# QEDProtocol/plonky2.5

Hardware: AMD Instinct MI355X
Metric: recursive proofs/sec (fib-64 p3-in-p2 circuit) (higher is better)
Workload: dtype u64 (Goldilocks, p = 2^64 - 2^32 + 1); 1 GPU; batch of 256 independent fib-64 plonky3-verifier proofs per GPU (n = 2^16 rows x 135 wires, LDE 2^19), 1 GPU(s), replicas + RCCL gather; all_statuses_ok=True, gathered_complete_and_ok=True, head=

## Files before the change

### plonky2.5_amd/csrc/capi.hip

```cpp
#include <stdlib.h>
#include <dirent.h>
#include <unistd.h>
#include <cstring>
#include <memory>
#include <atomic>
#include <mutex>
#include "../../include/p25.h"
#include "kernels.h"
#include "circuit_io.h"
#include "circuit_bytes.h"
#include "json_io.h"
#include "p3_circuit.h"
#include "p3_prover.h"
#include "p3_kernels.h"
#include "prover.h"
#include "recursion.h"

namespace p25 {
thread_local std::string g_last_error;
static std::atomic<int> g_device{-1};
static std::once_flag g_tables_once;
static std::unique_ptr<NttTables> g_tables;
static std::mutex g_primitives_mutex;

// ... 343 lines not shown
    bits -= a;
    if (deg < 0 || bits < (int)cap_height) return false;
  }
  return true;
}
}
}

using namespace p25;

extern "C" {

const char* p25_last_error(void) { return g_last_error.c_str(); }
const char* p25_version(void) { return "libp25 0.1 (gfx950)"; }

p25_status p25_device_init(int device_index) {
  const p25_status s = p25_device_init_ex(device_index, P25_DEFAULT_HW_QUEUES);
  return s == P25_WARN_HW_QUEUES_LATE ? P25_OK : s;
}

p25_status p25_device_init_ex(int device_index, int hw_queues) {
  if (hw_queues < 0 || hw_queues > P25_DEFAULT_HW_QUEUES) {
    g_last_error = "hw_queues out of range (0..2; 0 = leave the runtime's setting alone)";
    return P25_ERR_INVALID_ARG;
  }
  const bool late = apply_hw_queues(hw_queues);
  int n = 0;
  if (hipGetDeviceCount(&n) != hipSuccess || n <= 0) {
    g_last_error = "no HIP device available (libp25 has no CPU fallback)";
    return P25_ERR_NO_DEVICE;
  }
  if (device_index < 0 || device_index >= n) {
    g_last_error = "device index out of range";
    return P25_ERR_INVALID_ARG;
  }
  if (hipSetDevice(device_index) != hipSuccess) {
    g_last_error = "hipSetDevice failed";
    return P25_ERR_HIP;
  }
  g_device.store(device_index, std::memory_order_release);
  if (late) {
    g_last_error = HWQ_LATE_MSG;
    return P25_WARN_HW_QUEUES_LATE;
  }
  return P25_OK;
}

p25_status p25_runtime_info(p25_runtime_info_t* out) {
  if (!out) {
    g_last_error = "out is null";
    return P25_ERR_INVALID_ARG;
  }
  memset(out, 0, sizeof *out);
  out->device_index = g_device.load(std::memory_order_acquire);
  {
    std::lock_guard<std::mutex> l(g_hwq.mu);
    out->hw_queues_requested = g_hwq.requested;
    out->hw_queues_host_exported = g_hwq.host_exported ? 1 : 0;
    out->runtime_open_before_init = g_hwq.runtime_was_up ? 1 : 0;
    out->hw_queues_setting_late = (g_hwq.decided && g_hwq.requested > 0 && !g_hwq.host_exported && g_hwq.runtime_was_up) ? 1 : 0;
  }
  const char* e = getenv("GPU_MAX_HW_QUEUES");
  out->hw_queues_env = e ? (int32_t)strtol(e, nullptr, 10) : 0;
  out->proving_streams = 16;
  out->main_streams = 2;
  return P25_OK;
}

p25_status p25_poseidon_permute(uint64_t* states, size_t n) { return permute_host(states, n, launch_poseidon_permute, true); }
p25_status p25_poseidon2_permute(uint64_t* states, size_t n) { return permute_host(states, n, launch_poseidon2_permute, false); }

p25_status p25_merkle_commit(const uint64_t* leaves_cm, size_t n_leaves, size_t width,
                             unsigned cap_height, uint64_t* cap_out, uint64_t* tree_out) {
  return guarded([&]() -> p25_status {
    if (!is_pow2(n_leaves) || cap_height > 40 || n_leaves < ((size_t)1 << cap_height) || !width ||
        width > (1u << 20) || !leaves_cm)
      throw std::invalid_argument("p25_merkle_commit: bad shape");
    for (size_t i = 0; i < n_leaves * width; i++)
      if (leaves_cm[i] >= gl::P) throw std::invalid_argument("p25_merkle_commit: non-canonical field element");
    DevBuf d(n_leaves * width);
    size_t tw = merkle_tree_words(n_leaves, cap_height);
    DevBuf t(tw);
    P25_HIP(hipMemcpy(d.p, leaves_cm, n_leaves * width * 8, hipMemcpyHostToDevice));
    u64* cap = launch_merkle_tree(d.p, n_leaves, (int)width, n_leaves, cap_height, t.p, 0);
    P25_HIP(hipGetLastError());
    if (cap_out) P25_HIP(hipMemcpy(cap_out, cap, ((size_t)32) << cap_height, hipMemcpyDeviceToHost));
    if (tree_out) P25_HIP(hipMemcpy(tree_out, t.p, tw * 8, hipMemcpyDeviceToHost));
    P25_HIP(hipDeviceSynchronize());
    return P25_OK;
  });
}
size_t p25_merkle_tree_words(size_t n_leaves, unsigned cap_height) {
  if (!is_pow2(n_leaves) || cap_height > 63 || n_leaves < ((size_t)1 << cap_height)) return 0;
  return merkle_tree_words(n_leaves, cap_height);
}
p25_status p25_lde_commit(const uint64_t* polys, unsigned log_n, size_t n_polys, int from_coeffs,
                          unsigned rate_bits, unsigned cap_height, uint64_t* coeffs_out,
                          uint64_t* lde_out, uint64_t* cap_out) {
  return guarded([&]() -> p25_status {
    if (!polys || !n_polys || log_n > 20 || rate_bits > 3 || log_n + rate_bits < cap_height)
      throw std::invalid_argument("p25_lde_commit: bad shape");
    const size_t n = (size_t)1 << log_n, big = n << rate_bits;
    for (size_t i = 0; i < n * n_polys; i++)
      if (polys[i] >= gl::P) throw std::invalid_argument("p25_lde_commit: non-canonical field element");
    std::lock_guard<std::mutex> lk(g_primitives_mutex);
    DevBuf in(n * n_polys), co(n * n_polys), tmp(n * n_polys), lde(big * n_polys);
    size_t tw = merkle_tree_words(big, cap_height);
    DevBuf tree(tw);
    P25_HIP(hipMemcpy(in.p, polys, n * n_polys * 8, hipMemcpyHostToDevice));
    lde_commit_dev(in.p, log_n, n_polys, from_coeffs != 0, rate_bits, cap_height, co.p, tmp.p, lde.p,
                   tree.p, 0);
    P25_HIP(hipGetLastError());
    P25_HIP(hipDeviceSynchronize());
    if (coeffs_out)
      P25_HIP(hipMemcpy(coeffs_out, from_coeffs ? in.p : co.p, n * n_polys * 8, hipMemcpyDeviceToHost));
    if (lde_out) P25_HIP(hipMemcpy(lde_out, lde.p, big * n_polys * 8, hipMemcpyDeviceToHost));
    if (cap_out)
      P25_HIP(hipMemcpy(cap_out, tree.p + tw - ((size_t)4 << cap_height), ((size_t)32) << cap_height,
                        hipMemcpyDeviceToHost));
    return P25_OK;
  });
}
p25_status p25_merkle_commit_dev(const uint64_t* d_leaves_cm, size_t col_stride, size_t n_leaves,
                                 size_t width, unsigned cap_height, uint64_t* d_tree, void* stream) {
  return guarded([&]() -> p25_status {
    if (width > (1u << 20)) throw std::invalid_argument("p25_merkle_commit_dev: width above 2^20");
    if (!is_pow2(n_leaves) || cap_height > 40 || n_leaves < ((size_t)1 << cap_height) || !width ||
        col_stride < n_leaves || !d_leaves_cm || !d_tree)
      throw std::invalid_argument("p25_merkle_commit_dev: bad shape");
    launch_merkle_tree(d_leaves_cm, col_stride, (int)width, n_leaves, cap_height, d_tree,
                       (hipStream_t)stream);
    P25_HIP(hipGetLastError());
    return P25_OK;
  });
}
p25_status p25_lde_commit_dev(const uint64_t* d_polys, unsigned log_n, size_t n_polys, int from_coeffs,
                              unsigned rate_bits, unsigned cap_height, uint64_t* d_coeffs,
                              uint64_t* d_tmp, uint64_t* d_lde, uint64_t* d_tree, void* stream) {
  return guarded([&]() -> p25_status {
    if (log_n <= 20 && rate_bits <= 3 && cap_height > log_n + rate_bits)
      throw std::invalid_argument("p25_lde_commit_dev: cap_height above log_n + rate_bits");
    if (!d_polys || !n_polys || log_n > 20 || rate_bits > 3 || !d_lde ||
        (!from_coeffs && (!d_coeffs || !d_tmp)))
      throw std::invalid_argument("p25_lde_commit_dev: bad shape");
    std::lock_guard<std::mutex> lk(g_primitives_mutex);
    lde_commit_dev(d_polys, log_n, n_polys, from_coeffs != 0, rate_bits, cap_height, d_coeffs, d_tmp,
                   d_lde, d_tree, (hipStream_t)stream);
    P25_HIP(hipGetLastError());
    return P25_OK;
  });
}
p25_status p25_poseidon_permute_dev(uint64_t* d_states, size_t n, void* stream) {
  return guarded([&]() -> p25_status {
    launch_poseidon_permute(d_states, n, (hipStream_t)stream);
    P25_HIP(hipGetLastError());
    return P25_OK;
  });
}

p25_status p25_circuit_build_p3_verifier(const p25_p3_config* cfg, int32_t air, p25_circuit** out) {
  return host_guarded([&]() -> p25_status {
    if (!cfg || !out) throw std::invalid_argument("null argument");
    if (air != P25_AIR_FIBONACCI) throw std::invalid_argument("unknown AIR");
    FibonacciAir fib;
    return build_verifier(cfg, fib, out);
  });
}
// ... 520 lines not shown
```

### plonky2.5_amd/csrc/kernels.h

```cpp
#pragma once
#include <hip/hip_runtime.h>
#include <stddef.h>
#include <stdint.h>
#include <stdexcept>
#include <string>
#include <vector>
#include <map>
#include <tuple>
#include "gl.h"

#if defined(__HIP_DEVICE_COMPILE__)
#define P25_WAVE_PRIO(n) __builtin_amdgcn_s_setprio(n)
#else
#define P25_WAVE_PRIO(n) ((void)0)
#endif
#define P25_PRIO_BULK 2
#define P25_PRIO_CHAIN 3
namespace p25 {

struct HipError : std::runtime_error {
  using std::runtime_error::runtime_error;
};
#define P25_HIP(expr)                                                                         \
  do {                                                                                        \
    hipError_t _e = (expr);                                                                   \
    if (_e != hipSuccess)                                                                     \
      throw p25::HipError(std::string(#expr) + ": " + hipGetErrorString(_e) + " at " +        \
                          __FILE__ + ":" + std::to_string(__LINE__));                         \
  } while (0)

void launch_poseidon_permute(u64* d_states, size_t n, hipStream_t st);
void launch_poseidon2_permute(u64* d_states, size_t n, hipStream_t st);
size_t merkle_tree_words(size_t n_leaves, unsigned cap_height);
size_t merkle_level_offset(size_t n_leaves, unsigned level);
u64* launch_merkle_tree(const u64* d_cols, size_t col_stride, int width, size_t n_leaves,
                        unsigned cap_height, u64* d_tree, hipStream_t st, hipEvent_t ev_begin = nullptr,
                        hipEvent_t ev_end = nullptr, bool single_proof = false);

struct NttPass {
  const u64* in;
  u64* out;
  size_t in_poly_stride, out_poly_stride;
  size_t coset_out_off[8];
  int log_r, log_nt, log_t;
  int in_kind, in_br_t, in_br_i;
  int out_kind, out_br_t, out_br_i;
  const u64* pow_table;
  int log_n_table;
  int use_twiddle;
  const u64* pre;
  const u64* pre_t;
  const u64* pre_i;
  const u64* post_t;
  const u64* post_i;
  int inverse;
  int lazy_out;
  uint32_t n_tiles, n_cosets, log_g, full_table;
};
void launch_ntt_pass(const NttPass& p, int n_polys, int n_cosets, hipStream_t st);
double measure_shader_clock_hz(hipStream_t st);

class NttTables {
 public:
  ~NttTables();
  const u64* pow_table(int log_n, bool inverse);
  const u64* geom_table(u64 first, u64 ratio, size_t len);
  const u64* upload(const std::vector<u64>& host);
  typedef std::map<std::tuple<int, int, u64>, const u64*> CosetCache;
  CosetCache& coset_cache() { return coset_; }

 private:
  CosetCache coset_;
  std::map<std::pair<int, bool>, u64*> pow_;
  std::map<std::tuple<u64, u64, size_t>, u64*> geom_;
  std::vector<u64*> owned_;
};

void ntt_inverse(NttTables& tb, const u64* d_in, size_t in_stride, bool in_bitrev, u64* d_tmp,
                 size_t tmp_stride, u64* d_out, size_t out_stride, int log_n, int n_polys,
                 u64 coset_shift, hipStream_t st);
void ntt_lde_bitrev(NttTables& tb, const u64* d_coeffs, size_t coeff_stride, u64* d_lde,
                    size_t lde_stride, int log_n, int rate_bits, int n_polys, u64 shift,
                    hipStream_t st);

void ntt_inverse_then_lde(NttTables& tb, const u64* d_vals, size_t val_stride, u64* d_tmp, size_t tmp_stride, u64* d_coeffs,
                          size_t coeff_stride, u64* d_lde, size_t lde_stride, int log_n, int rate_bits, int n_polys, u64 shift,
                          hipStream_t st);

}
```

### plonky2.5_amd/csrc/kernels_hash.hip

```cpp
#include "kernels.h"
#include "poseidon.h"
#include "poseidon2.h"
#include "coop.h"
#include "coop_lat.h"

namespace p25 {

__global__ __launch_bounds__(256) void k_poseidon_permute(u64* states, size_t n) {
  size_t i = (size_t)blockIdx.x * blockDim.x + threadIdx.x;
  if (i >= n) return;
  u64 s[12];
#pragma unroll
  for (int k = 0; k < 12; k++) s[k] = states[i * 12 + k];
  poseidon::permute(s);
#pragma unroll
  for (int k = 0; k < 12; k++) states[i * 12 + k] = s[k];
}

__global__ __launch_bounds__(256) void k_poseidon2_permute(u64* states, size_t n) {
  size_t i = (size_t)blockIdx.x * blockDim.x + threadIdx.x;
  if (i >= n) return;
  u64 s[12];
#pragma unroll
  for (int k = 0; k < 12; k++) s[k] = states[i * 12 + k];
  poseidon2::permute(s);
#pragma unroll
  for (int k = 0; k < 12; k++) states[i * 12 + k] = s[k];
}

__device__ __forceinline__ void hash_leaf(const u64* __restrict__ cols, size_t col_stride, int width,
                                          size_t n_leaves, u64* __restrict__ digests) {
  size_t l = (size_t)blockIdx.x * 64 + threadIdx.x;
  if (l >= n_leaves) return;
  u64 out[4];
  poseidon::hash_or_noop_strided(cols + l, col_stride, width, out);
  u64* d = digests + 4 * l;
#pragma unroll
  for (int i = 0; i < 4; i++) d[i] = out[i];
}
__global__ __launch_bounds__(64, 6) void k_hash_leaves(const u64* __restrict__ cols, size_t col_stride,
                                                       int width, size_t n_leaves, u64* __restrict__ digests) {
  hash_leaf(cols, col_stride, width, n_leaves, digests);
}
__global__ __launch_bounds__(64, 6) void k_hash_leaves_wide(const u64* __restrict__ cols, size_t col_stride,
                                                            int width, size_t n_leaves, u64* __restrict__ digests) {
  hash_leaf(cols, col_stride, width, n_leaves, digests);
}

template <int PRIO>
__global__ __launch_bounds__(64, 8) void k_tree_level(const u64* __restrict__ children,
                                                    u64* __restrict__ parents, size_t n_parents) {
  if constexpr (PRIO != 0) P25_WAVE_PRIO(PRIO);
  size_t m = (size_t)blockIdx.x * 64 + threadIdx.x;
  if (m >= n_parents) return;
  u64 l[4], r[4], o[4];
#pragma unroll
  for (int i = 0; i < 4; i++) {
    l[i] = children[8 * m + i];
    r[i] = children[8 * m + 4 + i];
  }
  poseidon::two_to_one(l, r, o);
#pragma unroll
  for (int i = 0; i < 4; i++) parents[4 * m + i] = o[i];
}

__global__ __launch_bounds__(256) void k_tree_level_coop(const u64* __restrict__ children,
                                                         u64* __restrict__ parents, size_t n_parents) {
  P25_WAVE_PRIO(P25_PRIO_CHAIN);
  __shared__ u64 rc_lds[360];
  coop::stage_poseidon_rc(rc_lds);
  size_t g = ((size_t)blockIdx.x * blockDim.x + threadIdx.x) / coop::GROUP;
  const int rr = threadIdx.x & (coop::GROUP - 1);
  const bool valid = g < n_parents;
  if (!valid) g = n_parents - 1;
  u64 s = rr < 8 ? children[8 * g + rr] : 0;
  s = coop::poseidon_permute_lat(s, threadIdx.x & 63, rc_lds);
  if (valid && rr < 4) parents[4 * g + rr] = s;
}
constexpr int TOP_GROUPS = 16;
constexpr size_t TOP_MAX_NODES = 2 * TOP_GROUPS;
__global__ __launch_bounds__(256) void k_tree_top_coop(u64* __restrict__ nodes, uint32_t per_block, uint32_t n_blocks) {
  P25_WAVE_PRIO(P25_PRIO_CHAIN);
  __shared__ u64 rc_lds[360];
  __shared__ u64 lvl[2][TOP_GROUPS * 4];
  coop::stage_poseidon_rc(rc_lds);
  const int g = threadIdx.x / coop::GROUP, rr = threadIdx.x & (coop::GROUP - 1), lane = threadIdx.x & 63;
  const uint32_t b = blockIdx.x;
  u64* cur = nodes;
  size_t level_nodes = (size_t)per_block * n_blocks;
  uint32_t np = per_block >> 1;
  int buf = 0;
  bool first = true;
  while (np >= 1) {
    u64* nxt = cur + 4 * level_nodes;
    const uint32_t j = (uint32_t)g < np ? (uint32_t)g : np - 1;
    if ((uint32_t)(g & ~3) < np) {
      u64 s = 0;
      if (rr < 8) s = first ? cur[4 * ((size_t)b * 2 * np) + 8 * j + rr] : lvl[buf ^ 1][8 * j + rr];
      s = coop::poseidon_permute_lat(s, lane, rc_lds);
      if ((uint32_t)g < np && rr < 4) {
        nxt[4 * ((size_t)b * np + j) + rr] = s;
        lvl[buf][4 * j + rr] = s;
      }
    }
    __syncthreads();
    cur = nxt;
    level_nodes >>= 1;
    np >>= 1;
    buf ^= 1;
    first = false;
  }
}

constexpr size_t COOP_PARENTS_BATCH = 2048, COOP_PARENTS_SINGLE = 32768;
constexpr int LEVEL_PRIO_BATCH = 1;

static void launch_level(const u64* cur, u64* nxt, size_t m, hipStream_t st, bool single_proof) {
  const dim3 grid((unsigned)((m + 63) / 64));
  if (m <= (single_proof ? COOP_PARENTS_SINGLE : COOP_PARENTS_BATCH)) {
    size_t th = m * coop::GROUP;
    hipLaunchKernelGGL(k_tree_level_coop, dim3((unsigned)((th + 255) / 256)), dim3(256), 0, st, cur, nxt, m);
  } else if (single_proof) {
    hipLaunchKernelGGL(k_tree_level<0>, grid, dim3(64), 0, st, cur, nxt, m);
  } else {
    hipLaunchKernelGGL(k_tree_level<LEVEL_PRIO_BATCH>, grid, dim3(64), 0, st, cur, nxt, m);
  }
}
static u64* launch_levels_to_cap(u64* cur, size_t m, unsigned cap_height, hipStream_t st, bool single_proof) {
  const size_t cap = (size_t)1 << cap_height;
  while (m > cap) {
    if (m / cap <= TOP_MAX_NODES && cap <= 65536) {
      hipLaunchKernelGGL(k_tree_top_coop, dim3((unsigned)cap), dim3(TOP_GROUPS * coop::GROUP), 0, st, cur,
                         (uint32_t)(m / cap), (uint32_t)cap);
      while (m > cap) {
        cur += 4 * m;
        m >>= 1;
      }
      return cur;
    }
    u64* nxt = cur + 4 * m;
    m >>= 1;
    launch_level(cur, nxt, m, st, single_proof);
    cur = nxt;
  }
  return cur;
}

__global__ __launch_bounds__(64) void k_clock_probe(u64* sink, int reps, unsigned long long* clk) {
  size_t l = (size_t)blockIdx.x * blockDim.x + threadIdx.x;
  u64 s[12];
#pragma unroll
  for (int i = 0; i < 12; i++) s[i] = l * 12 + i;
  unsigned long long c0 = __builtin_readcyclecounter(), w0 = wall_clock64();
  for (int r = 0; r < reps; r++) {
    s[0] ^= (u64)r;
    poseidon::permute(s);
  }
  unsigned long long c1 = __builtin_readcyclecounter(), w1 = wall_clock64();
  if (s[0] == 0x123456789ull) sink[l & 63] = s[1];
  if (threadIdx.x == 0 && (blockIdx.x & 1023) == 0) {
    clk[2 * (blockIdx.x >> 10)] = c1 - c0;
    clk[2 * (blockIdx.x >> 10) + 1] = w1 - w0;
  }
}
double measure_shader_clock_hz(hipStream_t st) {
  const unsigned blocks = 8192, probes = blocks / 1024;
  u64* d = nullptr;
  P25_HIP(hipMalloc(&d, (64 + 2 * probes) * 8));
  unsigned long long* clk = (unsigned long long*)(d + 64);
  int dev = 0, khz = 0;
  P25_HIP(hipGetDevice(&dev));
  P25_HIP(hipDeviceGetAttribute(&khz, hipDeviceAttributeWallClockRate, dev));
  unsigned long long h[2 * probes];
  for (int it = 0; it < 2; it++)
    hipLaunchKernelGGL(k_clock_probe, dim3(blocks), dim3(64), 0, st, d, 64, clk);
  hipError_t e = hipMemcpyAsync(h, clk, sizeof(h), hipMemcpyDeviceToHost, st);
  if (e == hipSuccess) e = hipStreamSynchronize(st);
  (void)hipFree(d);
  P25_HIP(e);
  double cyc = 0, ticks = 0;
  for (unsigned i = 0; i < probes; i++) {
    cyc += (double)h[2 * i];
    ticks += (double)h[2 * i + 1];
  }
  if (ticks <= 0 || khz <= 0) return 0.0;
  return cyc / (ticks / ((double)khz * 1e3));
}

void launch_poseidon_permute(u64* d_states, size_t n, hipStream_t st) {
  if (!n) return;
  hipLaunchKernelGGL(k_poseidon_permute, dim3((unsigned)((n + 255) / 256)), dim3(256), 0, st, d_states, n);
}
void launch_poseidon2_permute(u64* d_states, size_t n, hipStream_t st) {
  if (!n) return;
  hipLaunchKernelGGL(k_poseidon2_permute, dim3((unsigned)((n + 255) / 256)), dim3(256), 0, st, d_states, n);
}

size_t merkle_tree_words(size_t n_leaves, unsigned cap_height) {
  size_t total = 0;
  for (size_t m = n_leaves; m >= ((size_t)1 << cap_height); m >>= 1) {
    total += 4 * m;
    if (m == 1) break;
  }
  return total;
}
size_t merkle_level_offset(size_t n_leaves, unsigned level) {
  size_t off = 0;
  size_t m = n_leaves;
  for (unsigned k = 0; k < level; k++) {
    off += 4 * m;
    m >>= 1;
  }
  return off;
}

u64* launch_merkle_tree(const u64* d_cols, size_t col_stride, int width, size_t n_leaves,
                        unsigned cap_height, u64* d_tree, hipStream_t st, hipEvent_t ev_begin,
                        hipEvent_t ev_end, bool single_proof) {
  if (ev_begin) (void)hipEventRecord(ev_begin, st);
  if (width >= 128)
    hipLaunchKernelGGL(k_hash_leaves_wide, dim3((unsigned)((n_leaves + 63) / 64)), dim3(64), 0, st, d_cols,
                       col_stride, width, n_leaves, d_tree);
  else
    hipLaunchKernelGGL(k_hash_leaves, dim3((unsigned)((n_leaves + 63) / 64)), dim3(64), 0, st, d_cols,
                       col_stride, width, n_leaves, d_tree);
  if (ev_end) (void)hipEventRecord(ev_end, st);
  return launch_levels_to_cap(d_tree, n_leaves, cap_height, st, single_proof);
}

void launch_tree_from_digests(u64* d_tree, size_t n_leaves, unsigned cap_height, hipStream_t st, bool single_proof) {
  launch_levels_to_cap(d_tree, n_leaves, cap_height, st, single_proof);
}

}
```

### plonky2.5_amd/csrc/prover.hip

```cpp
#include "prover.h"
#include <algorithm>
#include <map>
#include <mutex>
#include <string.h>
#include "poseidon.h"

namespace p25 {

constexpr size_t STREAM_POOL = 16;
namespace {
struct StreamPool {
  std::mutex mu;
  std::map<int, std::vector<hipStream_t>> per_device;
  size_t cursor = 0;
  size_t width = STREAM_POOL;
  size_t reserve(size_t count, size_t want_width) {
    std::lock_guard<std::mutex> l(mu);
    if (want_width > width) width = want_width;
    size_t first = cursor % width;
    cursor += count;
    return first;
  }
  void widen(size_t want_width) {
    std::lock_guard<std::mutex> l(mu);
// ... 104 lines not shown
  size_t m = (size_t)1 << log_n;
  const size_t nl = arity_bits.size();
  if (nl > 8) throw std::invalid_argument("too many FRI layers");
  for (size_t l = 0; l <= nl; l++) {
    coeffs[l] = DevMem(2 * m);
    if (l < nl) {
      size_t nvals = m << rate_bits;
      vals[l] = DevMem(2 * nvals);
      tree[l] = DevMem(merkle_tree_words(nvals >> arity_bits[l], cap_height));
      m >>= arity_bits[l];
    }
  }
}

void fri_commit_pow_query(NttTables& tables, FriWork& w, const FriShape& sh, Transcript* tr, u64* chal, QueryArgs qy,
                          u64* d_proof, const FriOffsets& fo, uint32_t* d_status, hipStream_t st, bool single_proof) {
  const size_t capw = (size_t)4 << sh.cap_height;
  size_t m = (size_t)1 << sh.log_n;
  int log_m = sh.log_n;
  u64 shift = gl::GENERATOR;
  const size_t nl = sh.arity_bits.size();
  for (size_t l = 0; l < nl; l++) {
    const int ab = sh.arity_bits[l];
    const size_t nvals = m << sh.rate_bits;
    ntt_lde_bitrev(tables, w.coeffs[l].p, m, w.vals[l].p, nvals, log_m, sh.rate_bits, 2, shift, st);
    const size_t n_leaves = nvals >> ab;
    launch_fri_leaf_hash(w.vals[l].p, w.vals[l].p + nvals, (uint32_t)n_leaves, ab, w.tree[l].p, st, single_proof);
    launch_tree_from_digests(w.tree[l].p, n_leaves, sh.cap_height, st, single_proof);
    const size_t ltw = merkle_tree_words(n_leaves, sh.cap_height);
    const u64* cap = w.tree[l].p + ltw - capw;
    {
      TranscriptArgs ta{};
      ta.seg[0] = TrSegment{cap, nullptr, d_proof + fo.caps + l * capw, (uint32_t)capw};
      ta.n_seg = 1;
      ta.chal_out = chal + CH_FRI_BETAS + 2 * l;
      ta.n_chal = 2;
      launch_transcript(tr, ta, st);
    }
    launch_fri_fold(w.coeffs[l].p, w.coeffs[l].p + m, (uint32_t)(m >> ab), ab, chal + CH_FRI_BETAS + 2 * l,
                    w.coeffs[l + 1].p, w.coeffs[l + 1].p + (m >> ab), st);
    qy.arity_bits[l] = ab;
    qy.layer_va[l] = w.vals[l].p;
    qy.layer_vb[l] = w.vals[l].p + nvals;
    qy.layer_tree[l] = w.tree[l].p;
    shift = gl::pow(shift, (u64)1 << ab);
    m >>= ab;
    log_m -= ab;
  }
  {
    TranscriptArgs ta{};
    ta.seg[0] = TrSegment{w.coeffs[nl].p, w.coeffs[nl].p + m, d_proof + fo.final_poly, (uint32_t)(2 * m)};
    ta.n_seg = 1;
    ta.close = TR_CLOSE_POW_INIT;
    ta.close_out = chal + CH_POW_WITNESS;
    launch_transcript(tr, ta, st);
  }
  qy.n_layers = (uint32_t)nl;
  launch_pow_search(tr, sh.pow_bits, chal + CH_POW_WITNESS, st, single_proof);
  {
    TranscriptArgs ta{};
    ta.seg[0] = TrSegment{chal + CH_POW_WITNESS, nullptr, d_proof + fo.pow_witness, 1};
    ta.n_seg = 1;
    ta.chal_out = chal + CH_POW_RESPONSE;
    ta.n_chal = 1 + (uint32_t)sh.num_queries;
    ta.close = TR_CLOSE_FINISH;
    ta.close_arg = (uint32_t)sh.pow_bits;
    ta.status = d_status;
    launch_transcript(tr, ta, st);
  }
  qy.chal = chal;
  qy.num_queries = sh.num_queries;
  qy.lde_bits = sh.log_n + sh.rate_bits;
  qy.cap_height = sh.cap_height;
  qy.proof = d_proof;
  qy.query_offset = (uint32_t)fo.queries;
  qy.query_stride = (uint32_t)fo.query_stride;
  launch_queries(qy, st);
}

struct DeviceCircuit::Ctx {
  DevMem wires_vals, wires_coeffs, tmp, wires_lde, wires_tree;
  DevMem zs_vals, zs_coeffs, zs_lde, zs_tree, zpp_chunk, zpp_tot, zpp_btot;
  DevMem q_vals, q_tmp, q_coeffs, q_lde, q_tree;
  DevMem transcript, chal, alpha_pows, eval_pows;
  DevMem preamble;
  DevMem fri_comp, fri_scan;
  FriWork fri;
  DevMem proof, status;
  hipEvent_t ev[12];
  hipStream_t st = nullptr;
  hipEvent_t done[2] = {nullptr, nullptr};
  hipEvent_t join = nullptr;
  bool have_events = false;
  ~Ctx() {
    if (have_events)
      for (auto& e : ev) (void)hipEventDestroy(e);
    for (auto& e : done)
      if (e) (void)hipEventDestroy(e);
    if (join) (void)hipEventDestroy(join);
  }
};

DeviceCircuit::DeviceCircuit(Circuit c) : c_(std::move(c)) {
  if (c_.cfg.num_challenges != 2 || c_.cfg.rate_bits > 3 || c_.gates.size() > 16)
    throw std::invalid_argument("unsupported circuit configuration");
  if (c_.fri_reduction_arity_bits.size() > 8) throw std::invalid_argument("too many FRI layers");
  if (c_.num_partial_products + 1 > MAX_CHUNKS || c_.cfg.num_routed_wires > MAX_ROUTED ||
      c_.cfg.num_challenges * (2 + c_.num_partial_products) >= ALPHA_POWS || c_.num_gate_constraints > ALPHA_POWS)
    throw std::invalid_argument("circuit exceeds the permutation-argument / quotient kernels' capacities");
  stream_ = g_stream_pool.main_acquire(main_lease_);
  layout_ = make_proof_layout(c_);
  const size_t n = c_.degree();
  const int ncs = (int)c_.constants_sigmas.size();
  WitnessProgram wp = build_witness_program(c_);
  auto up32 = [&](const std::vector<uint32_t>& v) {
    DevMem m((v.size() + 1) / 2 + 1);
    P25_HIP(hipMemcpy(m.p, v.data(), v.size() * 4, hipMemcpyHostToDevice));
    u64* p = m.p;
    owned_.push_back(std::move(m));
    return (uint32_t*)p;
  };
  {
    DevMem m(wp.gens.size() * sizeof(WitGen) / 8 + 1);
    P25_HIP(hipMemcpy(m.p, wp.gens.data(), wp.gens.size() * sizeof(WitGen), hipMemcpyHostToDevice));
    wp_.d_gens = (WitGen*)m.p;
    owned_.push_back(std::move(m));
  }
  wp_.d_args = up32(wp.args);
  wp_.d_input_slots = up32(wp.input_slots);
  wp_.d_input_first = up32(wp.input_first);
  wp_.d_wire_slot_cm = up32(wp.wire_slot_cm);
  wp_.level_start = wp.level_start;
  for (size_t l = 0; l + 1 < wp.level_start.size(); l++) {
    uint32_t b = wp.level_start[l], e = wp.level_start[l + 1];
    uint32_t kind = GEN_POSEIDON2, pb = e, pc = 0;
    for (int pass = 0; pass < 2 && !pc; pass++) {
      kind = pass == 0 ? GEN_POSEIDON2 : GEN_POSEIDON;
      for (uint32_t g = b; g < e; g++)
        if (wp.gens[g].kind == kind) {
          if (!pc) pb = g;
          pc++;
        }
    }
    wp_.level_p2_begin.push_back(pb);
    wp_.level_p2_count.push_back(pc);
    wp_.level_coop_kind.push_back(kind);
    for (uint32_t k = 0; k < pc; k++) {
      const WitGen& g = wp.gens[pb + k];
      if (g.kind != kind || g.n_deps != 13 || g.n_outs != 4 + 106 + 12 || g.arg_off != wp.gens[pb].arg_off + k * 135u)
        throw std::logic_error("witness program: permutation generators of a level are not laid out contiguously");
    }
    wp_.level_perm_arg_base.push_back(pc ? wp.gens[pb].arg_off : 0);
  }
  wp_.d_pi_slots = wp.pi_slots.empty() ? nullptr : up32(wp.pi_slots);
  wp_.n_public_inputs = (uint32_t)wp.pi_slots.size();
  wp_.n_inputs = (uint32_t)wp.input_slots.size();
  wp_.num_slots = wp.num_slots;
  wp_.num_random_fill = wp.num_random_fill;
  wp_.n_wire_elems = wp.wire_slot_cm.size();

  cs_vals_ = DevMem((size_t)ncs * n);
  for (int p = 0; p < ncs; p++)
    P25_HIP(hipMemcpy(cs_vals_.p + (size_t)p * n, c_.constants_sigmas[p].data(), n * 8, hipMemcpyHostToDevice));
  cs_coeffs_ = DevMem((size_t)ncs * n);
  cs_lde_ = DevMem((size_t)ncs * big());
  const size_t tw = merkle_tree_words(big(), c_.cfg.cap_height);
// ... 33 lines not shown
    int s = c_.selector_index[i];
    qa_proto_.gates[i] = GateEntry{(uint32_t)c_.gates[i], (uint32_t)s, (uint32_t)c_.groups[s].first, (uint32_t)c_.groups[s].second};
  }
  qa_proto_.num_selectors = c_.num_selectors;
  qa_proto_.num_wires = c_.cfg.num_wires;
  qa_proto_.num_routed = c_.cfg.num_routed_wires;
  qa_proto_.num_partial_products = c_.num_partial_products;
  qa_proto_.quotient_degree_factor = c_.cfg.max_quotient_degree_factor;
  qa_proto_.degree_bits = c_.degree_bits;
  qa_proto_.rate_bits = c_.cfg.rate_bits;
  {
    u64 g_pow_n = gl::exp_pow2(gl::GENERATOR, c_.degree_bits);
    u64 wr = gl::root_of_unity(c_.cfg.rate_bits);
    for (int k = 0; k < (1 << c_.cfg.rate_bits); k++) {
      qa_proto_.zh[k] = gl::sub(gl::mul(g_pow_n, gl::pow(wr, k)), 1);
      qa_proto_.zh_inv[k] = gl::inv(qa_proto_.zh[k]);
    }
  }
  l0_inv_ = DevMem(big());
  launch_l0_inv(qa_proto_.pow_big, c_.degree_bits, c_.cfg.rate_bits, l0_inv_.p, stream_);
  P25_HIP(hipStreamSynchronize(stream_));
  qa_proto_.l0_inv = l0_inv_.p;
}

DeviceCircuit::~DeviceCircuit() {
  for (auto& c : ctxs_)
    if (c->st) (void)hipStreamSynchronize(c->st);
  if (stream_) (void)hipStreamSynchronize(stream_);
  ctxs_.clear();
  for (auto& e : ev_witness_)
    if (e) (void)hipEventDestroy(e);
  for (auto& v : marks_)
    for (auto& e : v) (void)hipEventDestroy(e);
  if (ev_ext_) (void)hipEventDestroy(ev_ext_);
  if (ev_main_) (void)hipEventDestroy(ev_main_);
  for (auto* v : {&kstats_pending_, &kstats_free_})
    for (auto& pr : *v) {
      (void)hipEventDestroy(pr.first);
      (void)hipEventDestroy(pr.second);
    }
}

void DeviceCircuit::commitment_to_host(std::vector<u64>& coeffs, std::vector<u64>& lde, std::vector<u64>& tree) {
  sync();
  coeffs.resize(cs_coeffs_.words);
  lde.resize(cs_lde_.words);
  tree.resize(cs_tree_.words);
  P25_HIP(hipMemcpy(coeffs.data(), cs_coeffs_.p, coeffs.size() * 8, hipMemcpyDeviceToHost));
  P25_HIP(hipMemcpy(lde.data(), cs_lde_.p, lde.size() * 8, hipMemcpyDeviceToHost));
  P25_HIP(hipMemcpy(tree.data(), cs_tree_.p, tree.size() * 8, hipMemcpyDeviceToHost));
}

void DeviceCircuit::ensure_ctx(size_t count) {
  for (auto& e : ev_witness_)
    if (!e) P25_HIP(hipEventCreateWithFlags(&e, hipEventDisableTiming));
  while (ctxs_.size() < count) {
  ctxs_.emplace_back(new Ctx());
  Ctx& x = *ctxs_.back();
  if (ctxs_.size() == 1) pool_first_ = g_stream_pool.reserve(count, (size_t)streams_);
  else g_stream_pool.widen((size_t)streams_);
  x.st = g_stream_pool.at(pool_first_ + ctxs_.size() - 1);
  for (auto& e : x.done) P25_HIP(hipEventCreateWithFlags(&e, hipEventDisableTiming));
  const size_t n = c_.degree(), B = big();
  const int W = c_.cfg.num_wires, NC = c_.cfg.num_challenges, NP = c_.num_partial_products;
  const int nz = NC * (1 + NP), nq = NC * c_.cfg.max_quotient_degree_factor;
  const size_t tw = merkle_tree_words(B, c_.cfg.cap_height);
  x.wires_vals = DevMem((size_t)W * n);
  x.wires_coeffs = DevMem((size_t)W * n);
  x.tmp = DevMem((size_t)W * n);
  x.wires_lde = DevMem((size_t)W * B);
  x.wires_tree = DevMem(tw);
  x.zs_vals = DevMem((size_t)nz * n);
  x.zs_coeffs = DevMem((size_t)nz * n);
  x.zs_lde = DevMem((size_t)nz * B);
  x.zs_tree = DevMem(tw);
  x.zpp_chunk = DevMem((size_t)NC * (NP + 1) * n);
  x.zpp_tot = DevMem((size_t)NC * n);
  x.zpp_btot = DevMem((size_t)NC * ((n + 255) / 256) + 16);
  x.q_vals = DevMem((size_t)NC * B);
  x.q_tmp = DevMem((size_t)NC * B);
  x.q_coeffs = DevMem((size_t)NC * B);
  x.q_lde = DevMem((size_t)nq * B);
  x.q_tree = DevMem(tw);
  x.preamble = DevMem(8);
  P25_HIP(hipMemcpy(x.preamble.p, preamble_.p, 64, hipMemcpyDeviceToDevice));
  x.transcript = DevMem(sizeof(Transcript) / 8 + 1);
  x.chal = DevMem(CH_WORDS);
  x.alpha_pows = DevMem(2 * ALPHA_POWS);
  {
    x.eval_pows = DevMem(eval_scratch_words(2, (size_t)layout_.oracle_width[0] + W + nz + nq + NC, (uint32_t)c_.degree_bits));
  }
  x.fri_comp = DevMem(4 * n);
  size_t total_polys = layout_.oracle_width[0] + layout_.oracle_width[1] + layout_.oracle_width[2] + layout_.oracle_width[3];
  x.fri_scan = DevMem(2 * (total_polys + 1) + 8 * (n + 1) + 4 * ((n + 255) / 256) + 64);
  x.fri.alloc(c_.degree_bits, c_.cfg.rate_bits, c_.cfg.cap_height, c_.fri_reduction_arity_bits);
  x.proof = DevMem(layout_.total);
  x.status = DevMem(1);
  for (auto& e : x.ev) P25_HIP(hipEventCreate(&e));
  x.have_events = true;
  }
}

void DeviceCircuit::ensure_vals(int buf, size_t batch) {
  if (batch <= vals_batch_[buf]) return;
  sync();
  vals_[buf] = DevMem();
  vals_[buf] = DevMem((size_t)wp_.num_slots * batch);
  vals_batch_[buf] = batch;
}

void DeviceCircuit::sync() {
  P25_HIP(hipStreamSynchronize(stream_));
  for (auto& c : ctxs_) P25_HIP(hipStreamSynchronize(c->st));
}

void DeviceCircuit::stream_join(hipStream_t ext) {
  if (!ev_main_) P25_HIP(hipEventCreateWithFlags(&ev_main_, hipEventDisableTiming));
  P25_HIP(hipEventRecord(ev_main_, stream_));
  P25_HIP(hipStreamWaitEvent(ext, ev_main_, 0));
  for (auto& c : ctxs_) {
    if (!c->join) P25_HIP(hipEventCreateWithFlags(&c->join, hipEventDisableTiming));
    P25_HIP(hipEventRecord(c->join, c->st));
    P25_HIP(hipStreamWaitEvent(ext, c->join, 0));
  }
}
void DeviceCircuit::wait_stream(hipStream_t ext) {
  if (!ev_ext_) P25_HIP(hipEventCreateWithFlags(&ev_ext_, hipEventDisableTiming));
  P25_HIP(hipEventRecord(ev_ext_, ext));
  P25_HIP(hipStreamWaitEvent(stream_, ev_ext_, 0));
}

void DeviceCircuit::mark(int slot) {
  if (slot < 0 || slot >= MAX_MARKS) throw std::invalid_argument("mark slot out of range");
  auto& ev = marks_[slot];
  while (ev.size() < 1 + ctxs_.size()) {
    hipEvent_t e = nullptr;
    P25_HIP(hipEventCreateWithFlags(&e, hipEventDisableTiming));
    ev.push_back(e);
  }
  P25_HIP(hipEventRecord(ev[0], stream_));
  for (size_t k = 0; k < ctxs_.size(); k++) P25_HIP(hipEventRecord(ev[1 + k], ctxs_[k]->st));
  marks_recorded_[slot] = 1 + ctxs_.size();
}
void DeviceCircuit::stream_wait_mark(hipStream_t ext, int slot) {
  if (slot < 0 || slot >= MAX_MARKS) throw std::invalid_argument("mark slot out of range");
  for (size_t k = 0; k < marks_recorded_[slot]; k++) P25_HIP(hipStreamWaitEvent(ext, marks_[slot][k], 0));
}
void DeviceCircuit::wait_mark(DeviceCircuit& producer, int slot) {
  if (slot < 0 || slot >= MAX_MARKS) throw std::invalid_argument("mark slot out of range");
  for (size_t k = 0; k < producer.marks_recorded_[slot]; k++)
    P25_HIP(hipStreamWaitEvent(stream_, producer.marks_[slot][k], 0));
}

void DeviceCircuit::kernel_stats(double* ms, u64* launches, bool reset) {
  sync();
  for (auto& pr : kstats_pending_) {
    float t = 0;
    P25_HIP(hipEventElapsedTime(&t, pr.first, pr.second));
    kstats_ms_ += t;
    kstats_launches_++;
    kstats_free_.push_back(pr);
  }
  kstats_pending_.clear();
  if (ms) *ms = kstats_ms_;
  if (launches) *launches = kstats_launches_;
  if (reset) {
    kstats_ms_ = 0;
    kstats_launches_ = 0;
  }
}

void DeviceCircuit::prove_one(Ctx& x, int buf, size_t Bstride, uint32_t p, u64* d_proof,
                              uint32_t* d_status, PhaseTimes* t) {
  const u64* d_vals = vals_[buf].p;
  hipStream_t st = x.st;
  const size_t n = c_.degree(), B = big();
  const int W = c_.cfg.num_wires, NC = c_.cfg.num_challenges, NP = c_.num_partial_products;
  const int nz = NC * (1 + NP), nq = NC * c_.cfg.max_quotient_degree_factor;
  const int db = c_.degree_bits, rb = c_.cfg.rate_bits;
  const unsigned cap_h = c_.cfg.cap_height;
  const size_t capw = (size_t)4 << cap_h;
  const size_t tw = merkle_tree_words(B, cap_h);
  const ProofLayout& L = layout_;
  Transcript* tr = (Transcript*)x.transcript.p;
  u64* chal = x.chal.p;
  int evi = 0;
  auto mark = [&]() {
    if (t) P25_HIP(hipEventRecord(x.ev[evi++], st));
  };
  auto observe_cap = [&](const u64* cap, size_t proof_off, u64* chal_out, uint32_t n_chal, uint32_t close, uint32_t close_arg,
                         u64* close_out, bool with_preamble = false) {
    TranscriptArgs ta{};
    if (with_preamble) ta.seg[ta.n_seg++] = TrSegment{x.preamble.p, nullptr, nullptr, 8};
    ta.seg[ta.n_seg++] = TrSegment{cap, nullptr, d_proof + proof_off, (uint32_t)capw};
    ta.init = with_preamble;
    ta.chal_out = chal_out;
    ta.n_chal = n_chal;
    ta.close = close;
    ta.close_arg = close_arg;
    ta.close_out = close_out;
    ta.status = d_status;
    launch_transcript(tr, ta, st);
  };
  mark();
  launch_fill_wires(wp_, d_vals, Bstride, p, x.wires_vals.p, st);
  if (wp_.n_public_inputs)
    launch_public_inputs(d_vals, Bstride, p, wp_.d_pi_slots, wp_.n_public_inputs, d_proof + L.public_inputs, x.preamble.p + 4, st);
  P25_HIP(hipEventRecord(x.done[buf], st));
  mark();
  ntt_inverse_then_lde(tables_, x.wires_vals.p, n, x.tmp.p, n, x.wires_coeffs.p, n, x.wires_lde.p, B, db, rb, W, gl::GENERATOR, st);
  {
    hipEvent_t e0 = nullptr, e1 = nullptr;
    if (kstats_on_) {
      if (kstats_free_.empty()) {
        P25_HIP(hipEventCreate(&e0));
        P25_HIP(hipEventCreate(&e1));
      } else {
        e0 = kstats_free_.back().first;
        e1 = kstats_free_.back().second;
        kstats_free_.pop_back();
      }
      kstats_pending_.push_back({e0, e1});
    }
    launch_merkle_tree(x.wires_lde.p, B, W, B, cap_h, x.wires_tree.p, st, e0, e1, single_proof_);
  }
  const u64* wires_cap = x.wires_tree.p + tw - capw;
  observe_cap(wires_cap, L.wires_cap, chal + CH_BETAS, 2 * NC, TR_CLOSE_NONE, 0, nullptr, true);
  mark();
  enqueue_partial_products(x, st);
  mark();
  ntt_inverse_then_lde(tables_, x.zs_vals.p, n, x.tmp.p, n, x.zs_coeffs.p, n, x.zs_lde.p, B, db, rb, nz, gl::GENERATOR, st);
  launch_merkle_tree(x.zs_lde.p, B, nz, B, cap_h, x.zs_tree.p, st, nullptr, nullptr, single_proof_);
  const u64* zs_cap = x.zs_tree.p + tw - capw;
  observe_cap(zs_cap, L.zs_cap, chal + CH_ALPHAS, NC, TR_CLOSE_ALPHA_POWS, 0, x.alpha_pows.p);
  mark();
  enqueue_quotient(x, st, false);
  mark();
  ntt_lde_bitrev(tables_, x.q_coeffs.p, n, x.q_lde.p, B, db, rb, nq, gl::GENERATOR, st);
  launch_merkle_tree(x.q_lde.p, B, nq, B, cap_h, x.q_tree.p, st, nullptr, nullptr, single_proof_);
  const u64* q_cap = x.q_tree.p + tw - capw;
  observe_cap(q_cap, L.quotient_cap, chal + CH_ZETA, 2, TR_CLOSE_CHECK_ZETA, (uint32_t)db, nullptr);
  mark();
  {
    const u64 g = gl::root_of_unity(db);
    const EvalJob jobs[6] = {{cs_coeffs_.p, d_proof + L.constants, L.oracle_width[0], 0},
                             {x.wires_coeffs.p, d_proof + L.wires, (uint32_t)W, 0},
                             {x.zs_coeffs.p, d_proof + L.zs, (uint32_t)NC, 0},
                             {x.zs_coeffs.p + (size_t)NC * n, d_proof + L.pps, (uint32_t)(NC * NP), 0},
                             {x.q_coeffs.p, d_proof + L.quotient, (uint32_t)nq, 0},
                             {x.zs_coeffs.p, d_proof + L.zs_next, (uint32_t)NC, 1}};
    const u64 scales[2] = {1, g};
    launch_eval_jobs(jobs, 6, db, chal + CH_ZETA, scales, 2, x.eval_pows.p, st);
    {
      TranscriptArgs ta{};
      ta.seg[0] = TrSegment{d_proof + L.constants, nullptr, nullptr, (uint32_t)(L.zs_next - L.constants)};
      ta.seg[1] = TrSegment{d_proof + L.pps, nullptr, nullptr, (uint32_t)(L.fri_caps - L.pps)};
      ta.seg[2] = TrSegment{d_proof + L.zs_next, nullptr, nullptr, (uint32_t)(L.pps - L.zs_next)};
      ta.n_seg = 3;
      ta.chal_out = chal + CH_FRI_ALPHA;
      ta.n_chal = 2;
      launch_transcript(tr, ta, st);
    }
    mark();
    FriCombineArgs fa;
    fa.coeffs[0] = cs_coeffs_.p;
    fa.coeffs[1] = x.wires_coeffs.p;
    fa.coeffs[2] = x.zs_coeffs.p;
    fa.coeffs[3] = x.q_coeffs.p;
    for (int k = 0; k < 4; k++) fa.n_polys[k] = L.oracle_width[k];
    fa.log_n = db;
    fa.num_challenges = NC;
    fa.chal = chal;
    fa.g = g;
    fa.comp = x.fri_comp.p;
    fa.scan_tmp = x.fri_scan.p;
    fa.final_a = x.fri.coeffs[0].p;
    fa.final_b = x.fri.coeffs[0].p + n;
    launch_fri_combine(fa, st);
  }
  {
    QueryArgs qy;
    memset(&qy, 0, sizeof(qy));
    const u64* ldes[4] = {cs_lde_.p, x.wires_lde.p, x.zs_lde.p, x.q_lde.p};
    const u64* trees[4] = {cs_tree_.p, x.wires_tree.p, x.zs_tree.p, x.q_tree.p};
    qy.n_oracles = 4;
    for (int k = 0; k < 4; k++) {
      qy.oracle_lde[k] = ldes[k];
      qy.oracle_tree[k] = trees[k];
      qy.oracle_width[k] = L.oracle_width[k];
    }
    FriShape sh{db, rb, cap_h, c_.fri_reduction_arity_bits, c_.cfg.proof_of_work_bits, c_.cfg.num_query_rounds};
    FriOffsets fo{L.fri_caps, L.final_poly, L.pow_witness, L.queries, L.query_stride};
    fri_commit_pow_query(tables_, x.fri, sh, tr, chal, qy, d_proof, fo, d_status, st, single_proof_);
  }
  mark();
  P25_HIP(hipGetLastError());
  if (t) {
    P25_HIP(hipEventSynchronize(x.ev[8]));
    float ms[8];
    for (int i = 0; i < 8; i++) P25_HIP(hipEventElapsedTime(&ms[i], x.ev[i], x.ev[i + 1]));
    t->witness += ms[0];
    t->wires_commit += ms[1];
    t->zs_pp += ms[2];
    t->zs_commit += ms[3];
    t->quotient += ms[4];
    t->quotient_commit += ms[5];
    t->openings += ms[6];
    t->fri += ms[7];
    float tot;
    P25_HIP(hipEventElapsedTime(&tot, x.ev[0], x.ev[8]));
    t->total += tot;
  }
}

void DeviceCircuit::enqueue_partial_products(Ctx& x, hipStream_t st) {
  const size_t n = c_.degree();
  const int NC = c_.cfg.num_challenges, NP = c_.num_partial_products, db = c_.degree_bits;
  u64* chal = x.chal.p;
  {
    ZppArgs za;
    za.wires = x.wires_vals.p;
    za.sigmas = cs_vals_.p + (size_t)(c_.num_selectors + c_.cfg.num_constants) * n;
// ... 304 lines not shown
```

Before: 131.6 proofs/s.

## Fuse lower Merkle levels into leaf hashing via atomic last-arriver climb

Leaf-hashing kernels now continue up the Merkle tree: each 64-lane wave, after writing its leaf digests, atomically increments a per-parent counter, and the second arriver hashes the parent level and keeps climbing. The number of climbed levels is chosen so the remaining levels are handled by the existing coop/top kernels. This is meant to remove separate per-level launches and the extra global round trips for the large bottom levels. In exchange it adds atomics, fences and divergent wave exits, and it relies on counters self-resetting to zero so the buffer can be reused across commits.

```diff
diff --git a/plonky2.5_amd/csrc/capi.hip b/plonky2.5_amd/csrc/capi.hip
--- a/plonky2.5_amd/csrc/capi.hip
+++ b/plonky2.5_amd/csrc/capi.hip
@@ -449,7 +449,9 @@
     size_t tw = merkle_tree_words(n_leaves, cap_height);
     DevBuf t(tw);
     P25_HIP(hipMemcpy(d.p, leaves_cm, n_leaves * width * 8, hipMemcpyHostToDevice));
-    u64* cap = launch_merkle_tree(d.p, n_leaves, (int)width, n_leaves, cap_height, t.p, 0);
+    DevBuf cnt((merkle_climb_counter_words(n_leaves) * sizeof(uint32_t) + 15) / 16 * 2);
+    if (cnt.p) P25_HIP(hipMemset(cnt.p, 0, (merkle_climb_counter_words(n_leaves) * sizeof(uint32_t) + 15) / 16 * 16));
+    u64* cap = launch_merkle_tree(d.p, n_leaves, (int)width, n_leaves, cap_height, t.p, 0, nullptr, nullptr, false, (uint32_t*)cnt.p);
     P25_HIP(hipGetLastError());
     if (cap_out) P25_HIP(hipMemcpy(cap_out, cap, ((size_t)32) << cap_height, hipMemcpyDeviceToHost));
     if (tree_out) P25_HIP(hipMemcpy(tree_out, t.p, tw * 8, hipMemcpyDeviceToHost));
diff --git a/plonky2.5_amd/csrc/kernels.h b/plonky2.5_amd/csrc/kernels.h
--- a/plonky2.5_amd/csrc/kernels.h
+++ b/plonky2.5_amd/csrc/kernels.h
@@ -35,7 +35,9 @@
 size_t merkle_level_offset(size_t n_leaves, unsigned level);
 u64* launch_merkle_tree(const u64* d_cols, size_t col_stride, int width, size_t n_leaves,
                         unsigned cap_height, u64* d_tree, hipStream_t st, hipEvent_t ev_begin = nullptr,
-                        hipEvent_t ev_end = nullptr, bool single_proof = false);
+                        hipEvent_t ev_end = nullptr, bool single_proof = false, uint32_t* d_climb_cnt = nullptr);
+constexpr size_t MERKLE_CLIMB_WAVE_LEAVES = 64;
+inline size_t merkle_climb_counter_words(size_t n_leaves) { return n_leaves / MERKLE_CLIMB_WAVE_LEAVES; }
 
 struct NttPass {
   const u64* in;
diff --git a/plonky2.5_amd/csrc/kernels_hash.hip b/plonky2.5_amd/csrc/kernels_hash.hip
--- a/plonky2.5_amd/csrc/kernels_hash.hip
+++ b/plonky2.5_amd/csrc/kernels_hash.hip
@@ -45,6 +45,62 @@
 __global__ __launch_bounds__(64, 6) void k_hash_leaves_wide(const u64* __restrict__ cols, size_t col_stride,
                                                             int width, size_t n_leaves, u64* __restrict__ digests) {
   hash_leaf(cols, col_stride, width, n_leaves, digests);
+}
+
+constexpr int LEVEL_PRIO_BATCH = 1;
+__device__ __forceinline__ void climb_levels(u64* tree, uint32_t* cnt, uint32_t n_waves, int n_climb) {
+  P25_WAVE_PRIO(LEVEL_PRIO_BATCH);
+  const uint32_t lane = threadIdx.x;
+  uint32_t task = blockIdx.x, tasks = n_waves;
+  u64* cur = tree;
+  size_t m = (size_t)n_waves * 64;
+  for (int k = 1; k <= n_climb; k++) {
+    task >>= 1;
+    tasks >>= 1;
+    asm volatile("s_waitcnt vmcnt(0)" ::: "memory");
+    uint32_t prev = 0;
+    if (lane == 0) {
+      __builtin_amdgcn_fence(__ATOMIC_RELEASE, "agent");
+      asm volatile("s_waitcnt vmcnt(0)" ::: "memory");
+      prev = __hip_atomic_fetch_add(cnt + task, 1u, __ATOMIC_RELAXED, __HIP_MEMORY_SCOPE_AGENT);
+    }
+    prev = (uint32_t)__builtin_amdgcn_readfirstlane((int)prev);
+    if (prev == 0) return;
+    if (lane == 0) __hip_atomic_store(cnt + task, 0u, __ATOMIC_RELAXED, __HIP_MEMORY_SCOPE_AGENT);
+    __builtin_amdgcn_fence(__ATOMIC_ACQUIRE, "agent");
+    u64* nxt = cur + 4 * m;
+    const size_t p = (size_t)task * 64 + lane;
+    u64 l[4], r[4], o[4];
+#pragma unroll
+    for (int i = 0; i < 4; i++) {
+      l[i] = cur[8 * p + i];
+      r[i] = cur[8 * p + 4 + i];
+    }
+    poseidon::two_to_one(l, r, o);
+#pragma unroll
+    for (int i = 0; i < 4; i++) nxt[4 * p + i] = o[i];
+    cur = nxt;
+    m >>= 1;
+    cnt += tasks;
+  }
+}
+__device__ __forceinline__ void hash_leaf_climb(const u64* __restrict__ cols, size_t col_stride, int width, u64* tree,
+                                                uint32_t* cnt, uint32_t n_waves, int n_climb) {
+  const size_t l = (size_t)blockIdx.x * 64 + threadIdx.x;
+  u64 out[4];
+  poseidon::hash_or_noop_strided(cols + l, col_stride, width, out);
+  u64* d = tree + 4 * l;
+#pragma unroll
+  for (int i = 0; i < 4; i++) d[i] = out[i];
+  climb_levels(tree, cnt, n_waves, n_climb);
+}
+__global__ __launch_bounds__(64, 6) void k_hash_leaves_climb(const u64* __restrict__ cols, size_t col_stride, int width,
+                                                             u64* tree, uint32_t* cnt, uint32_t n_waves, int n_climb) {
+  hash_leaf_climb(cols, col_stride, width, tree, cnt, n_waves, n_climb);
+}
+__global__ __launch_bounds__(64, 6) void k_hash_leaves_wide_climb(const u64* __restrict__ cols, size_t col_stride, int width,
+                                                                  u64* tree, uint32_t* cnt, uint32_t n_waves, int n_climb) {
+  hash_leaf_climb(cols, col_stride, width, tree, cnt, n_waves, n_climb);
 }
 
 template <int PRIO>
@@ -113,7 +169,6 @@
 }
 
 constexpr size_t COOP_PARENTS_BATCH = 2048, COOP_PARENTS_SINGLE = 32768;
-constexpr int LEVEL_PRIO_BATCH = 1;
 
 static void launch_level(const u64* cur, u64* nxt, size_t m, hipStream_t st, bool single_proof) {
   const dim3 grid((unsigned)((m + 63) / 64));
@@ -214,18 +269,36 @@
   return off;
 }
 
+static int climbed_levels(size_t n_leaves, unsigned cap_height) {
+  const size_t cap = (size_t)1 << cap_height;
+  int k = 0;
+  for (size_t m = n_leaves; m > cap && !(m / cap <= TOP_MAX_NODES && cap <= 65536) && (m >> 1) > COOP_PARENTS_BATCH; m >>= 1) k++;
+  return k;
+}
+
 u64* launch_merkle_tree(const u64* d_cols, size_t col_stride, int width, size_t n_leaves,
                         unsigned cap_height, u64* d_tree, hipStream_t st, hipEvent_t ev_begin,
-                        hipEvent_t ev_end, bool single_proof) {
+                        hipEvent_t ev_end, bool single_proof, uint32_t* d_climb_cnt) {
+  const bool pow2 = n_leaves && !(n_leaves & (n_leaves - 1));
+  const int n_climb = (d_climb_cnt && !single_proof && pow2 && n_leaves <= ((size_t)1 << 37)) ? climbed_levels(n_leaves, cap_height) : 0;
   if (ev_begin) (void)hipEventRecord(ev_begin, st);
-  if (width >= 128)
+  if (n_climb) {
+    const uint32_t n_waves = (uint32_t)(n_leaves / 64);
+    if (width >= 128)
+      hipLaunchKernelGGL(k_hash_leaves_wide_climb, dim3(n_waves), dim3(64), 0, st, d_cols, col_stride, width, d_tree,
+                         d_climb_cnt, n_waves, n_climb);
+    else
+      hipLaunchKernelGGL(k_hash_leaves_climb, dim3(n_waves), dim3(64), 0, st, d_cols, col_stride, width, d_tree,
+                         d_climb_cnt, n_waves, n_climb);
+  } else if (width >= 128)
     hipLaunchKernelGGL(k_hash_leaves_wide, dim3((unsigned)((n_leaves + 63) / 64)), dim3(64), 0, st, d_cols,
                        col_stride, width, n_leaves, d_tree);
   else
     hipLaunchKernelGGL(k_hash_leaves, dim3((unsigned)((n_leaves + 63) / 64)), dim3(64), 0, st, d_cols,
                        col_stride, width, n_leaves, d_tree);
   if (ev_end) (void)hipEventRecord(ev_end, st);
-  return launch_levels_to_cap(d_tree, n_leaves, cap_height, st, single_proof);
+  return launch_levels_to_cap(d_tree + merkle_level_offset(n_leaves, (unsigned)n_climb), n_leaves >> n_climb, cap_height, st,
+                              single_proof);
 }
 
 void launch_tree_from_digests(u64* d_tree, size_t n_leaves, unsigned cap_height, hipStream_t st, bool single_proof) {
diff --git a/plonky2.5_amd/csrc/prover.hip b/plonky2.5_amd/csrc/prover.hip
--- a/plonky2.5_amd/csrc/prover.hip
+++ b/plonky2.5_amd/csrc/prover.hip
@@ -210,6 +210,7 @@
   DevMem wires_vals, wires_coeffs, tmp, wires_lde, wires_tree;
   DevMem zs_vals, zs_coeffs, zs_lde, zs_tree, zpp_chunk, zpp_tot, zpp_btot;
   DevMem q_vals, q_tmp, q_coeffs, q_lde, q_tree;
+  DevMem climb_cnt;
   DevMem transcript, chal, alpha_pows, eval_pows;
   DevMem preamble;
   DevMem fri_comp, fri_scan;
@@ -409,6 +410,8 @@
   x.q_coeffs = DevMem((size_t)NC * B);
   x.q_lde = DevMem((size_t)nq * B);
   x.q_tree = DevMem(tw);
+  x.climb_cnt = DevMem((merkle_climb_counter_words(B) * sizeof(uint32_t) + 7) / 8);
+  P25_HIP(hipMemsetAsync(x.climb_cnt.p, 0, x.climb_cnt.words * 8, x.st));
   x.preamble = DevMem(8);
   P25_HIP(hipMemcpy(x.preamble.p, preamble_.p, 64, hipMemcpyDeviceToDevice));
   x.transcript = DevMem(sizeof(Transcript) / 8 + 1);
@@ -549,7 +552,7 @@
       }
       kstats_pending_.push_back({e0, e1});
     }
-    launch_merkle_tree(x.wires_lde.p, B, W, B, cap_h, x.wires_tree.p, st, e0, e1, single_proof_);
+    launch_merkle_tree(x.wires_lde.p, B, W, B, cap_h, x.wires_tree.p, st, e0, e1, single_proof_, (uint32_t*)x.climb_cnt.p);
   }
   const u64* wires_cap = x.wires_tree.p + tw - capw;
   observe_cap(wires_cap, L.wires_cap, chal + CH_BETAS, 2 * NC, TR_CLOSE_NONE, 0, nullptr, true);
@@ -557,14 +560,14 @@
   enqueue_partial_products(x, st);
   mark();
   ntt_inverse_then_lde(tables_, x.zs_vals.p, n, x.tmp.p, n, x.zs_coeffs.p, n, x.zs_lde.p, B, db, rb, nz, gl::GENERATOR, st);
-  launch_merkle_tree(x.zs_lde.p, B, nz, B, cap_h, x.zs_tree.p, st, nullptr, nullptr, single_proof_);
+  launch_merkle_tree(x.zs_lde.p, B, nz, B, cap_h, x.zs_tree.p, st, nullptr, nullptr, single_proof_, (uint32_t*)x.climb_cnt.p);
   const u64* zs_cap = x.zs_tree.p + tw - capw;
   observe_cap(zs_cap, L.zs_cap, chal + CH_ALPHAS, NC, TR_CLOSE_ALPHA_POWS, 0, x.alpha_pows.p);
   mark();
   enqueue_quotient(x, st, false);
   mark();
   ntt_lde_bitrev(tables_, x.q_coeffs.p, n, x.q_lde.p, B, db, rb, nq, gl::GENERATOR, st);
-  launch_merkle_tree(x.q_lde.p, B, nq, B, cap_h, x.q_tree.p, st, nullptr, nullptr, single_proof_);
+  launch_merkle_tree(x.q_lde.p, B, nq, B, cap_h, x.q_tree.p, st, nullptr, nullptr, single_proof_, (uint32_t*)x.climb_cnt.p);
   const u64* q_cap = x.q_tree.p + tw - capw;
   observe_cap(q_cap, L.quotient_cap, chal + CH_ZETA, 2, TR_CLOSE_CHECK_ZETA, (uint32_t)db, nullptr);
   mark();
```

New measurement: 101.6 proofs/s. 0.772x the previous value.
